# zkwebauthn/webauthn-halo2

Hardware: AMD Instinct MI355X
Metric: webauthn_es256_proofs_per_sec_k19 (higher is better)
Workload: dtype u256-montgomery (9x29-bit carry-free limbs in the hot kernels: bucket accumulation, NTT, reduction tails, quotient; 8x32-bit limbs elsewhere and in memory)

## Files before the change

include/zkmi355.h:

```cpp
#ifndef ZKMI355_H
#define ZKMI355_H

#include <stddef.h>
#include <stdint.h>

#ifdef __cplusplus
extern "C" {
#endif

#define ZK_OK 0
#define ZK_EINVAL (-1)
#define ZK_ENOMEM (-2)
#define ZK_EHIP (-3)
#define ZK_ENODEV (-4)
#define ZK_ESTATE (-5)
#define ZK_EWITNESS (-6)
#define ZK_EINTERNAL (-7)
#define ZK_ELAYOUT (-8)

typedef struct zk_ctx zk_ctx;
typedef uint64_t zk_poly;

#define ZK_BASIS_MONOMIAL 0
#define ZK_BASIS_LAGRANGE 1
// ... 4 lines not shown
void* zk_host_alloc(size_t bytes);
void zk_host_free(void* p);
int zk_ctx_create(int device_id, zk_ctx** out);
int zk_ctx_create_shared(zk_ctx* parent, zk_ctx** out);
void zk_ctx_destroy(zk_ctx* ctx);
const char* zk_strerror(int code);
int zk_last_hip_error(const zk_ctx* ctx);
int zk_sync(zk_ctx* ctx);
#define ZK_OPT_MSM_WINDOW 1
#define ZK_OPT_MSM_BATCH 2
#define ZK_OPT_NTT_MAX_RADIX_LOG2 3
#define ZK_OPT_GP_BATCH_INVERT 4
#define ZK_OPT_MSM_TAIL_STREAM 5
#define ZK_OPT_MSM_TAIL_MAIN_ABOVE 6
#define ZK_OPT_BATCH_PASS_COLUMNS 7
#define ZK_OPT_XFORM_STREAM 8
#define ZK_OPT_MSM_STREAM 9
#define ZK_OPT_MSM_T1 10
#define ZK_OPT_STREAM_AUDIT 11
#define ZK_OPT_STREAM_PRIORITY 12
#define ZK_OPT_QUOTIENT_DOMAIN 13
#define ZK_OPT_ACTIVITY_HOLD 14
int zk_ctx_set_option(zk_ctx* ctx, int option, int64_t value);

int zk_msm_bn254(zk_ctx* ctx, const uint64_t* scalars_mont ,
                 const uint64_t* bases_affine_mont , size_t n,
                 uint64_t out_jacobian_mont[12]);
int zk_msm_srs(zk_ctx* ctx, int basis , const uint64_t* scalars_mont , size_t n,
               uint64_t out_jacobian_mont[12]);
int zk_ntt_bn254_fr(zk_ctx* ctx, uint64_t* a_mont , const uint64_t omega_mont[4],
                    uint32_t log_n);

int zk_srs_setup(zk_ctx* ctx, uint32_t k, const uint8_t seed[32]);
int zk_srs_load(zk_ctx* ctx, uint32_t k, const uint64_t* g, const uint64_t* g_lagrange);
int zk_srs_export(zk_ctx* ctx, int basis, uint64_t* out_affine_mont , size_t first, size_t count);
int zk_srs_k(const zk_ctx* ctx);
int zk_srs_msm_plan(const zk_ctx* ctx, uint32_t* window_bits, uint32_t* windows);

#define ZK_SERDE_PROCESSED 0
#define ZK_SERDE_RAW_BYTES 1
#define ZK_SERDE_RAW_BYTES_UNCHECKED 2
int zk_srs_write(zk_ctx* ctx, int format, uint8_t* out, size_t cap, size_t* len);
int zk_srs_read(zk_ctx* ctx, const uint8_t* bytes, size_t len, int format);
int zk_srs_set_g2(zk_ctx* ctx, const uint64_t g2[16], const uint64_t s_g2[16]);

int zk_g_to_lagrange(zk_ctx* ctx, const uint64_t* g , uint32_t k, uint64_t* out );
// ... 225 lines not shown
```

webauthn-halo2_amd/csrc/ctx.h:

```cpp
#pragma once
#include <map>
#include <memory>
#include <new>
#include <mutex>
#include <unordered_map>
#include <vector>

#include "../../include/zkmi355.h"
#include "engine.h"
#include "activity.h"
#include "audit.h"
#include "hostutil.h"

using namespace zk;

struct zk_pk_rec;

struct PolyRec {
    Fr* ptr;
    size_t n;
};

struct SrsBlock {
    int device = -1;
// ... 30 lines not shown
    bool audit_fault = false;
    std::mutex mu;
    std::map<uint32_t, Fr*> twiddles;
    std::map<uint32_t, Fr*> coset_points;
    std::map<uint32_t, Fr*> twiddles_ntt;
    std::map<uint32_t, Fr> ninv;
    std::map<uint32_t, Fr*> twiddles_ninv;
    std::map<uint32_t, Fr*> coset3_pre;
    std::map<uint32_t, Coset3Consts> coset3_consts;
    uint32_t opt_verify_inst_eval = 0;
    uint32_t opt_quotient_domain = 0;
    uint64_t srs_gen = 0;
    uint32_t opt_msm_window = 0, opt_msm_batch = 0, opt_ntt_max_r = 0, opt_gp_batch_invert = 0;
    uint32_t opt_tail_stream = 0;
    uint32_t opt_tail_main_above = 0;
    uint32_t opt_batch_pass_cols = 0;
    uint32_t msm_min_cols = 0;
    activity::State act;
    hipStream_t tail_stream = nullptr;
    hipStream_t msm_stream = nullptr;
    hipEvent_t ev_msm_in = nullptr;
    bool msm_side = false;
    uint32_t opt_msm_stream = 0;
    uint32_t opt_msm_t1 = 0;
    hipStream_t xform_stream = nullptr;
    hipEvent_t ev_rows = nullptr, ev_xform = nullptr;
    bool xform_pending = false;
    uint32_t opt_xform_stream = 0;
    uint64_t stream_counts[4] = {0, 0, 0, 0};
    static constexpr int MSM_LANES = 3;
    struct MsmLane {
        MsmWorkspace* ws = nullptr;
        MsmWorkspace* ws_gen = nullptr;
        MsmWorkspace* ws_run = nullptr;
        hipStream_t tail = nullptr;
        hipEvent_t head_done = nullptr, tail_done = nullptr;
        hipEvent_t t_head[2] = {nullptr, nullptr};
        hipEvent_t t_acc[4] = {nullptr, nullptr, nullptr, nullptr};
        size_t n = 0;
        const G1Affine* table = nullptr;
        G1X* host_buf = nullptr;
        bool busy = false;
        uint32_t nwin = 0, cw = 0;
        uint32_t batch = 1;
        bool fixed = false;
    } lanes[MSM_LANES];
// ... 132 lines not shown
```

webauthn-halo2_amd/csrc/ctx.hip:

```cpp
#include <stdlib.h>

#include <algorithm>
#include <new>

#include "ctx.h"
#include "prover.h"

namespace zk {
G1Affine g1_jac_to_affine_host(const G1Jac& p) {
    G1Affine r;
    if (p.z.is_zero()) {
        r.x = Fq::zero();
        r.y = Fq::zero();
        return r;
    }
    const Fq zi = fe_inv_fast(p.z);
    const Fq zi2 = fe_sqr(zi);
    r.x = fe_mul(p.x, zi2);
    r.y = fe_mul(p.y, fe_mul(zi2, zi));
    return r;
}
}

int ctx_bind(zk_ctx* c) {
    hipError_t e = hipSetDevice(c->device);
    if (e != hipSuccess) {
        c->last_hip = (int)e;
        return ZK_EHIP;
    }
// ... 129 lines not shown
}

const char* zk_strerror(int code) {
    switch (code) {
        case ZK_OK: return "ok";
        case ZK_EINVAL: return "invalid argument";
        case ZK_ENOMEM: return "out of memory";
        case ZK_EHIP: return "HIP runtime error";
        case ZK_ENODEV: return "no usable gfx950 device";
        case ZK_ESTATE: return "missing prerequisite (SRS / key not loaded)";
        case ZK_EWITNESS: return "witness does not satisfy the circuit (lookup input outside the table)";
        case ZK_EINTERNAL: return "internal error (C++ exception stopped at the ABI boundary)";
        case ZK_ELAYOUT: return "selector columns outside the layout of compress_selectors the key is built for";
        default: return "unknown error";
    }
}

ZK_API(zk_ctx_create, (int device_id, zk_ctx** out), (device_id, out)) {
    if (!out) return ZK_EINVAL;
    if (int rc = device_id_ok(device_id)) return rc;
    zk_ctx* c = new (std::nothrow) zk_ctx();
    if (!c) return ZK_ENOMEM;
    c->device = device_id;
    if (hipSetDevice(device_id) != hipSuccess ||
        ((c->stream_slot = pool_take_slot(device_id, &c->stream)) < 0 && hipStreamCreate(&c->stream) != hipSuccess) ||
        hipHostMalloc(&c->host_small, 8 * sizeof(Fr)) != hipSuccess ||
        hipMalloc(&c->small, (2048 + 8) * sizeof(Fr)) != hipSuccess) {
        zk_ctx_destroy(c);
        return ZK_EHIP;
    }
    for (int i = 0; i < ZK_T_COUNT; i++)
        if (hipEventCreate(&c->ev[i][0]) != hipSuccess || hipEventCreate(&c->ev[i][1]) != hipSuccess) {
            zk_ctx_destroy(c);
            return ZK_EHIP;
        }
    bool ok = true;
    for (hipEvent_t* e : {&c->ev_msm_in, &c->ev_rows, &c->ev_xform}) ok = ok && hipEventCreateWithFlags(e, hipEventDisableTiming) == hipSuccess;
    for (int i = 0; i < zk_ctx::MSM_LANES && ok; i++) {
        zk_ctx::MsmLane& L = c->lanes[i];
        L.tail = c->stream;
        for (hipEvent_t& e : L.t_head) ok = ok && hipEventCreate(&e) == hipSuccess;
        for (hipEvent_t& e : L.t_acc) ok = ok && hipEventCreate(&e) == hipSuccess;
        for (hipEvent_t* e : {&L.head_done, &L.tail_done}) ok = ok && hipEventCreateWithFlags(e, hipEventDisableTiming) == hipSuccess;
        ok = ok && hipHostMalloc(&L.host_buf, (size_t)MSM_MAX_BATCH * 15 * 4 * sizeof(G1X)) == hipSuccess;
    }
    if (!ok) {
// ... 5 lines not shown
    ctx_activity_register(c);
    *out = c;
    return ZK_OK;
}

ZK_API(zk_ctx_create_shared, (zk_ctx* parent, zk_ctx** out), (parent, out)) {
    if (!parent || !out) return ZK_EINVAL;
    zk_ctx* c = nullptr;
    int rc = zk_ctx_create(parent->device, &c);
    if (rc) return rc;
    std::lock_guard<std::mutex> lk(parent->mu);
    if (parent->srs_k >= 0) {
        static_cast<SrsView&>(*c) = *parent;
        c->opt_msm_window = parent->opt_msm_window;
        c->opt_msm_batch = parent->opt_msm_batch;
        c->opt_ntt_max_r = parent->opt_ntt_max_r;
        c->opt_gp_batch_invert = parent->opt_gp_batch_invert;
        c->opt_tail_stream = parent->opt_tail_stream;
        c->opt_tail_main_above = parent->opt_tail_main_above;
        c->opt_batch_pass_cols = parent->opt_batch_pass_cols;
        c->opt_xform_stream = parent->opt_xform_stream;
        c->opt_msm_stream = parent->opt_msm_stream;
        c->opt_msm_t1 = parent->opt_msm_t1;
        c->srs_gen++;
    }
    *out = c;
    return ZK_OK;
}

void zk_ctx_destroy(zk_ctx* c) {
    if (!c) return;
    ctx_activity_unregister(c);
    hipSetDevice(c->device);
    if (c->stream) aud_sync(c, c->stream);
    if (c->tail_stream) aud_sync(c, c->tail_stream);
    if (c->xform_stream) aud_sync(c, c->xform_stream);
    if (c->msm_stream) aud_sync(c, c->msm_stream);
    for (auto& kv : c->twiddles) hipFree(kv.second);
    for (auto& kv : c->twiddles_ntt) hipFree(kv.second);
    for (auto& kv : c->twiddles_ninv) hipFree(kv.second);
    for (auto& kv : c->coset_points) hipFree(kv.second);
    for (auto& kv : c->coset3_pre) hipFree(kv.second);
    pk_destroy_all(c);
    for (auto& kv : c->polys) hipFree(kv.second.ptr);
    for (auto& r : c->poly_spare) hipFree(r.ptr);
    c->srs.reset();
// ... 128 lines not shown
    *total_ms = c->acc_ms[which];
    *count = c->acc_n[which];
    return ZK_OK;
}

namespace {
struct PlainOption {
    int option;
    int64_t min, max;
    uint32_t zk_ctx::*member;
};
const PlainOption PLAIN_OPTIONS[] = {
    {ZK_OPT_MSM_WINDOW, 9, 17, &zk_ctx::opt_msm_window},
    {ZK_OPT_MSM_TAIL_STREAM, 0, 2, &zk_ctx::opt_tail_stream},
    {ZK_OPT_MSM_TAIL_MAIN_ABOVE, 0, 64, &zk_ctx::opt_tail_main_above},
    {ZK_OPT_MSM_STREAM, 0, 2, &zk_ctx::opt_msm_stream},
    {ZK_OPT_MSM_T1, 0, 2, &zk_ctx::opt_msm_t1},
    {ZK_OPT_XFORM_STREAM, 0, 2, &zk_ctx::opt_xform_stream},
    {ZK_OPT_BATCH_PASS_COLUMNS, 0, MSM_MAX_BATCH, &zk_ctx::opt_batch_pass_cols},
    {ZK_OPT_MSM_BATCH, 0, MSM_MAX_BATCH, &zk_ctx::opt_msm_batch},
    {ZK_OPT_NTT_MAX_RADIX_LOG2, 1, 11, &zk_ctx::opt_ntt_max_r},
    {ZK_OPT_QUOTIENT_DOMAIN, 0, 2, &zk_ctx::opt_quotient_domain},
};
}

ZK_API(zk_ctx_set_option, (zk_ctx* c, int option, int64_t value), (c, option, value)) {
    if (!c || value < 0) return ZK_EINVAL;
    std::lock_guard<std::mutex> lk(c->mu);
    for (const PlainOption& o : PLAIN_OPTIONS)
        if (o.option == option) {
            if (value && (value < o.min || value > o.max)) return ZK_EINVAL;
            c->*o.member = (uint32_t)value;
            return ZK_OK;
        }
    switch (option) {
        case ZK_OPT_STREAM_AUDIT:
            if (value > 2) return ZK_EINVAL;
            c->audit.reset();
            c->audit.streams[0] = c->stream;
            c->audit.on = value != 0;
            c->audit_fault = value == 2;
            return ZK_OK;
        case ZK_OPT_GP_BATCH_INVERT:
            c->opt_gp_batch_invert = value ? 1 : 0;
            return ZK_OK;
        case ZK_OPT_ACTIVITY_HOLD:
// ... 27 lines not shown
```

webauthn-halo2_amd/csrc/pk.h:

```cpp
#pragma once
#include <utility>
#include <vector>

#include "ctx.h"
#include "prover.h"

inline int resolve_scheme(int transcript, int* scheme) {
    if (transcript != ZK_TRANSCRIPT_BLAKE2B && transcript != ZK_TRANSCRIPT_EVM) return ZK_EINVAL;
    if (*scheme == ZK_SCHEME_DEFAULT) *scheme = transcript == ZK_TRANSCRIPT_EVM ? ZK_SCHEME_GWC : ZK_SCHEME_SHPLONK;
    return *scheme == ZK_SCHEME_GWC || *scheme == ZK_SCHEME_SHPLONK ? ZK_OK : ZK_EINVAL;
}

enum ColType { COL_ADVICE = 0, COL_FIXED = 1, COL_INSTANCE = 2 };
struct Col {
    int type;
    uint32_t idx;
};

struct Layout {
    uint32_t k, n, A, L, F, lookup_bits, idle;
    uint32_t n_inst;
    bool single;
    uint32_t n_gate, n_lookup_cols, n_adv, fx_table, fx_qlookup, n_fix;
    std::vector<uint32_t> fx_sel;
// ... 73 lines not shown
static constexpr uint32_t BATCH_ARGS_MIN = 8;
static constexpr uint32_t ROWS_CAP = 512, ROWS_BLOCKS = 16;

struct zk_pk_rec {
    Layout lay;
    uint64_t srs_gen = 0;
    std::vector<Fr*> dev;
    std::vector<Fr*> fixed_val, fixed_poly, fixed_coset, sigma_val, sigma_poly, sigma_coset;
    Fr *l0_coset = nullptr, *l_last_coset = nullptr, *l_active_coset = nullptr;
    std::vector<Fr*> fixed_c3, sigma_c3;
    Fr *l0_c3 = nullptr, *l_last_c3 = nullptr, *l_active_c3 = nullptr;
    std::vector<G1Affine> fixed_commit, perm_commit;
    Fr transcript_repr;
    bool verify_only = false;
    G1Affine* d_vk_bases = nullptr;
    std::vector<Fr*> adv_val, adv_poly, adv_coset;
    Fr *inst_val = nullptr, *inst_poly = nullptr, *inst_coset = nullptr;
    std::vector<Fr*> z_val, z_poly, z_coset;
    std::vector<Fr*> lk_in, lk_ap, lk_ap_poly, lk_ap_coset, lk_sp, lk_sp_poly, lk_sp_coset, lk_z, lk_z_poly, lk_z_coset,
        lk_in_coset;
    Fr *random_poly = nullptr, *h_ext = nullptr, *h_comb = nullptr;
    Fr *t_num = nullptr, *t_den = nullptr, *t_frac = nullptr, *t_a = nullptr, *t_b = nullptr, *t_small = nullptr;
    Fr* kd_scratch = nullptr;
    Fr* tail_host = nullptr;
    RowEntry* rows_host = nullptr;
    RowEntry* rows_dev = nullptr;
    LookupScratch lks{};
    uint32_t* lk_u32 = nullptr;
    std::vector<Fr*> gp_num, gp_den, gp_loc_p, gp_loc_r;
    Fr* gp_tot = nullptr;
    Fr* gp_scal = nullptr;
    Fr* gp_host = nullptr;
    GpItem* d_gp_items = nullptr;
    void *h_batch_args = nullptr, *d_batch_args = nullptr;
    size_t batch_args_bytes = 0;
    QuotientArgs* d_qargs = nullptr;
    QuotientArgs* h_qargs = nullptr;
    EvalItem *d_evargs = nullptr, *h_evargs = nullptr;
    Fr t_inv[4];
    bool t_inv_ready = false;
    uint32_t max_evals = 0;
    LcTerm *d_lc_terms = nullptr, *h_lc_terms = nullptr;
    uint32_t lc_cap = 0, lc_used = 0;
    Fr *ev_scratch = nullptr, *ev_out = nullptr;
    bool is_member = false;
    std::vector<zk_pk_rec*> members;
// ... 61 lines not shown
```

webauthn-halo2_amd/csrc/prover.hip:

```cpp
#include <stdlib.h>

#include <algorithm>
#include <deque>
#include <functional>
#include <memory>
#include <unordered_map>
#include <vector>

#include "prover_steps.h"

using namespace zk;

#ifdef ZK_HOST_TRACE
#include <chrono>
#include <cstdio>
static std::chrono::steady_clock::time_point& ht_last() {
    static thread_local std::chrono::steady_clock::time_point t = std::chrono::steady_clock::now();
    return t;
}
#define HT(name)                                                                                                  \
    do {                                                                                                          \
        const auto ht_now = std::chrono::steady_clock::now();                                                     \
        fprintf(stderr, "HT %-24s +%7.1f us\n", name, std::chrono::duration<double, std::micro>(ht_now - ht_last()).count()); \
        ht_last() = ht_now;                                                                                       \
    } while (0)
#else
#define HT(name) do { } while (0)
#endif


namespace {
// ... 580 lines not shown
    }

    struct CR {
        const Fr* poly;
        std::vector<int> rots;
        std::vector<Fr> evals;
    };
    struct RotPt {
        int rot;
        Fr pt, canon;
    };
    struct RS {
        std::vector<int> rots;
        std::vector<size_t> coms;
    };
    struct Shplonk {
        std::vector<CR> com;
        std::vector<RotPt> rot_pts;
        std::vector<RS> rsets;
        std::vector<int> all_rots;
        std::vector<std::vector<Fr>> low;
        Fr yc, v;
        Fr* hx = nullptr;
    };
    static const RotPt& sh_rot_pt(const Shplonk& S, int r) {
        for (auto& e : S.rot_pts)
            if (e.rot == r) return e;
        return S.rot_pts[0];
    }
    int shplonk_stage1(const std::vector<Q>& queries, const Fr& x, Shplonk& S) {
        std::vector<CR>& com = S.com;
        {
            std::unordered_map<const Fr*, size_t> seen;
            seen.reserve(queries.size());
            for (auto& qq : queries) {
                auto it = seen.find(qq.poly);
                if (it == seen.end()) {
                    it = seen.emplace(qq.poly, com.size()).first;
                    com.push_back(CR{qq.poly, {}, {}});
                }
                com[it->second].rots.push_back(qq.rot);
                com[it->second].evals.push_back(qq.eval);
            }
        }
        for (auto& qq : queries) {
            bool have = false;
// ... 22 lines not shown
                r2.push_back(cr.rots[i]);
                e2.push_back(cr.evals[i]);
            }
            cr.rots = r2;
            cr.evals = e2;
            for (int r : cr.rots)
                if (std::find(all_rots.begin(), all_rots.end(), r) == all_rots.end()) all_rots.push_back(r);
            size_t hit = rsets.size();
            for (size_t si = 0; si < rsets.size(); si++)
                if (rsets[si].rots == cr.rots) hit = si;
            if (hit == rsets.size()) rsets.push_back(RS{cr.rots, {}});
            rsets[hit].coms.push_back(ci);
        }
        std::sort(all_rots.begin(), all_rots.end(), pt_less);
        HT("grouped");
        S.yc = tr->squeeze();
        S.v = tr->squeeze();
        const Fr yc = S.yc, v = S.v;
        S.low.assign(com.size(), {});
        Fr* hx = pk->t_frac;
        S.hx = hx;
        Fr* sbuf[6] = {pk->h_ext, pk->h_ext + n, pk->h_ext + 2 * (size_t)n, pk->h_ext + 3 * (size_t)n, pk->t_num, pk->t_den};
        if (rsets.size() > 6) return ZK_ESTATE;
        std::vector<std::vector<Fr>> set_pts;
        size_t max_pts = 0;
        for (size_t si = 0; si < rsets.size(); si++) {
            auto& rs = rsets[si];
            std::vector<Fr> pts;
            for (int r : rs.rots) pts.push_back(sh_rot_pt(S, r).pt);
            const std::vector<std::vector<Fr>> basis = lagrange_basis(pts);
            std::vector<Term> terms;
            std::vector<Fr> rsum(pts.size(), Fr::zero());
            Fr py = Fr::one();
            for (size_t ci : rs.coms) {
                const CR& cr = com[ci];
                std::vector<Fr>& lo = S.low[ci];
                lo.assign(pts.size(), Fr::zero());
                for (size_t j = 0; j < pts.size(); j++)
                    for (size_t t = 0; t < pts.size(); t++) lo[t] = fe_add(lo[t], fe_mul(basis[j][t], cr.evals[j]));
                terms.push_back(Term{cr.poly, py});
                for (size_t t = 0; t < pts.size(); t++) rsum[t] = fe_add(rsum[t], fe_mul(py, lo[t]));
                py = fe_mul(py, yc);
            }
            if (pts.size() > 8) return ZK_ESTATE;
            lincomb_many(sbuf[si], terms, false, Fr::zero(), false, &rsum);
        HT("set lincomb launched");
            max_pts = std::max(max_pts, pts.size());
            set_pts.push_back(pts);
        }
        for (size_t step = 0; step < max_pts; step++) {
            Fr* bufs[6];
            Fr zs[6];
            uint32_t cnt = 0;
            for (size_t si = 0; si < rsets.size(); si++)
                if (step < set_pts[si].size()) {
                    bufs[cnt] = sbuf[si];
                    zs[cnt] = set_pts[si][step];
                    cnt++;
                }
            if (c->audit.on) {
                std::vector<const void*> b(bufs, bufs + cnt);
                AV(b, b, "SHPLONK: division step");
            }
            launch_kate_division_batch(bufs, bufs, zs, cnt, n, pk->kd_scratch, st);
        }
        {
            std::vector<Term> terms;
            Fr pv = Fr::one();
            for (size_t si = 0; si < rsets.size(); si++) {
                terms.push_back(Term{sbuf[si], pv});
                pv = fe_mul(pv, v);
            }
            lincomb_many(hx, terms, false, Fr::zero());
        HT("hx launched");
        }
        return rc;
    }
    int shplonk_stage2(Shplonk& S, const Fr** out) {
        const Fr u = tr->squeeze();
        HT("u squeezed");
        std::vector<Term> terms;
        Fr sub = Fr::zero();
        Fr pv = Fr::one();
        std::vector<Fr> z_diffs;
        for (auto& rs : S.rsets) {
            std::vector<Fr> diffs;
            for (int r : S.all_rots)
                if (std::find(rs.rots.begin(), rs.rots.end(), r) == rs.rots.end()) diffs.push_back(sh_rot_pt(S, r).pt);
            const Fr zi = vanishing_eval(diffs, u);
            z_diffs.push_back(zi);
            Fr py = Fr::one();
            for (size_t ci : rs.coms) {
                const Fr coef = fe_mul(fe_mul(pv, zi), py);
                terms.push_back(Term{S.com[ci].poly, coef});
                sub = fe_add(sub, fe_mul(coef, eval_small(S.low[ci], u)));
                py = fe_mul(py, S.yc);
            }
            pv = fe_mul(pv, S.v);
        }
        std::vector<Fr> all_pts;
        for (int r : S.all_rots) all_pts.push_back(sh_rot_pt(S, r).pt);
        const Fr zt = vanishing_eval(all_pts, u);
        terms.push_back(Term{S.hx, fe_neg(zt)});
        lincomb_many(pk->t_a, terms, true, sub);
        HT("L launched");
        A({pk->t_a}, {pk->t_b}, "SHPLONK: final division");
        launch_kate_division(pk->t_a, pk->t_b, n, u, pk->kd_scratch, st);
        A({pk->t_b}, {pk->t_b}, "SHPLONK: scale");
        launch_scale(pk->t_b, fe_inv_fast(z_diffs[0]), n, st);
        *out = pk->t_b;
        return rc;
    }
    int open_shplonk(const std::vector<Q>& queries, const Fr& x) {
        Shplonk S;
        if (int r = shplonk_stage1(queries, x, S)) return r;
        commit_write(S.hx, ZK_BASIS_MONOMIAL);
        if (!ok()) return rc;
        const Fr* last = nullptr;
        if (int r = shplonk_stage2(S, &last)) return r;
        commit_write(last, ZK_BASIS_MONOMIAL);
        return rc;
    }
};

#include "prover_lockstep.h"

}

namespace {
struct ProveQuiesce {
    zk_ctx* c;
    explicit ProveQuiesce(zk_ctx* ctx) : c(ctx) { ctx_activity_hold(c, true); }
// ... 234 lines not shown
```

webauthn-halo2_amd/csrc/prover_key.hip:

```cpp
#include <stdlib.h>

#include <algorithm>
#include <unordered_map>
#include <vector>

#include "pk.h"
#include "vkrepr.h"

using namespace zk;

namespace {

__global__ void sigma_kernel(const uint2* __restrict__ map, const Fr* __restrict__ tw, const Fr* __restrict__ dpow,
                             Fr* __restrict__ out, uint32_t n) {
    const uint32_t i = blockIdx.x * blockDim.x + threadIdx.x;
    if (i >= n) return;
    const uint2 m = map[i];
    fe_store(out + i, fe_mul(fe_load(dpow + m.x), fe_load(tw + m.y)));
}

bool commit(zk_ctx* c, const Fr* poly, size_t len, int basis, G1Affine* out) {
    G1Jac j;
    if (ctx_msm_device(c, poly, ctx_basis(c, basis), len, &j) != ZK_OK) return false;
    *out = g1_jac_to_affine_host(j);
// ... 84 lines not shown
    }
    for (uint32_t l = 0; l < lay.n_lookups; l++) {
        pk->lk_in.push_back(lay.single ? d.alloc(n) : nullptr);
        pk->lk_ap.push_back(d.alloc(n));
        pk->lk_ap_poly.push_back(d.alloc(n));
        pk->lk_ap_coset.push_back(d.alloc(N));
        pk->lk_sp.push_back(d.alloc(n));
        pk->lk_sp_poly.push_back(d.alloc(n));
        pk->lk_sp_coset.push_back(d.alloc(N));
        pk->lk_z.push_back(d.alloc(n));
        pk->lk_z_poly.push_back(d.alloc(n));
        pk->lk_z_coset.push_back(d.alloc(N));
    }
    pk->random_poly = d.alloc(n);
    pk->h_ext = d.alloc(N);
    pk->h_comb = d.alloc(n);
    pk->t_num = d.alloc(n);
    pk->t_den = d.alloc(n);
    pk->t_frac = d.alloc(n);
    pk->t_a = d.alloc(n);
    pk->t_b = d.alloc(n);
    pk->t_small = d.alloc(n / 16 + 8192);
    pk->kd_scratch = d.alloc((size_t)KD_MAX_BATCH * kate_division_scratch(n));
    {
        const uint32_t nprod = lay.n_chunks + lay.n_lookups;
        for (uint32_t p = 0; p < nprod; p++) {
            pk->gp_num.push_back(d.alloc(n));
            pk->gp_den.push_back(d.alloc(n));
            pk->gp_loc_p.push_back(d.alloc(n));
            pk->gp_loc_r.push_back(d.alloc(n));
        }
        pk->gp_tot = d.alloc((size_t)2 * gp_blocks(n) * nprod);
        pk->gp_scal = d.alloc((size_t)4 * nprod);
        if (hipHostMalloc(&pk->gp_host, (size_t)2 * nprod * sizeof(Fr)) != hipSuccess ||
            hipMalloc(&pk->d_gp_items, nprod * sizeof(GpItem)) != hipSuccess)
            return fail(ZK_ENOMEM);
    }
    if (d.rc) return fail(d.rc);
    if (hipHostMalloc(&pk->tail_host, (pk->max_evals + 16) * sizeof(Fr)) != hipSuccess) return fail(ZK_ENOMEM);
    if (hipHostMalloc(&pk->rows_host, (size_t)ROWS_BLOCKS * ROWS_CAP * sizeof(RowEntry)) != hipSuccess ||
        hipMalloc(&pk->rows_dev, (size_t)ROWS_BLOCKS * ROWS_CAP * sizeof(RowEntry)) != hipSuccess)
        return fail(ZK_ENOMEM);
    if (hipHostMalloc(&pk->h_evargs, pk->max_evals * sizeof(EvalItem)) != hipSuccess ||
        hipMalloc(&pk->d_evargs, pk->max_evals * sizeof(EvalItem)) != hipSuccess)
        return fail(ZK_ENOMEM);
    pk->lc_cap = 2 * (pk->max_evals + 8);
// ... 24 lines not shown
        bytes = std::max(bytes, (size_t)lay.n_lookups * sizeof(LkNumDenArgs));
        bytes = std::max(bytes, (size_t)lay.n_adv * sizeof(CopyPair));
        pk->batch_args_bytes = bytes;
        if (hipMalloc(&pk->d_batch_args, bytes) != hipSuccess || hipHostMalloc(&pk->h_batch_args, bytes) != hipSuccess) return fail(ZK_ENOMEM);
    }
    return ZK_OK;
}

static zk_pk_rec* pk_make_member(zk_ctx* c, const zk_pk_rec* pk) {
    zk_pk_rec* m = new (std::nothrow) zk_pk_rec(*pk);
    if (!m) return nullptr;
    m->is_member = true;
    m->dev.clear();
    m->members.clear();
    m->bb = nullptr;
    m->wc = nullptr;
    m->pc = nullptr;
    for (auto* v : {&m->adv_val, &m->adv_poly, &m->adv_coset, &m->z_val, &m->z_poly, &m->z_coset, &m->lk_in, &m->lk_ap, &m->lk_ap_poly,
                    &m->lk_ap_coset, &m->lk_sp, &m->lk_sp_poly, &m->lk_sp_coset, &m->lk_z, &m->lk_z_poly, &m->lk_z_coset, &m->lk_in_coset,
                    &m->gp_num, &m->gp_den, &m->gp_loc_p, &m->gp_loc_r})
        v->clear();
    m->inst_val = m->inst_poly = m->inst_coset = nullptr;
    m->random_poly = m->h_ext = m->h_comb = m->t_num = m->t_den = m->t_frac = m->t_a = m->t_b = m->t_small = m->kd_scratch = nullptr;
    m->tail_host = nullptr;
    m->rows_host = m->rows_dev = nullptr;
    m->lk_u32 = nullptr;
    m->gp_tot = m->gp_scal = m->gp_host = nullptr;
    m->d_gp_items = nullptr;
    m->h_batch_args = m->d_batch_args = nullptr;
    m->d_qargs = m->h_qargs = nullptr;
    m->d_evargs = m->h_evargs = nullptr;
    m->d_lc_terms = m->h_lc_terms = nullptr;
    m->ev_scratch = m->ev_out = nullptr;
    m->lc_used = 0;
    if (pk_alloc_workspace(c, m) != ZK_OK) {
        pk_destroy(m);
        return nullptr;
    }
    return m;
}

int pk_ensure_batch(zk_ctx* c, zk_pk_rec* pk, uint32_t batch) {
    if (batch <= 1) return ZK_OK;
    const Layout& lay = pk->lay;
    const uint32_t n = lay.n, T = 1u << lay.lookup_bits, nprod = lay.n_chunks + lay.n_lookups;
    if ((pk->members.size() + 1 < batch || !pk->bb || pk->bb->cap < batch) && !c->poly_spare.empty()) ctx_release_spares(c);
// ... 574 lines not shown
```

webauthn-halo2_amd/ecdsa_p256.py:

```python
import dataclasses
import hashlib
import os
import queue
import threading
import time

import numpy as np

from . import circuit
from .engine import (ZK_PK_CHECK_ALL, ZK_SCHEME_GWC, ZK_SCHEME_SHPLONK, ZK_SERDE_RAW_BYTES, ZK_SRS_CONTRIB_LINKS,
                     ZK_SRS_CONTRIB_NONTRIVIAL, ZK_SRS_CONTRIB_RESIDENT, ZK_SRS_CONTRIB_SAME_SECRET, ZK_TRANSCRIPT_BLAKE2B,
                     ZK_ES256_BATCH_MAX, ZK_TRANSCRIPT_EVM, Engine, ZkError, stream_placement)

_STATE = {}
_SLOTS_LOCK = threading.Lock()
_STATE_LOCK = threading.RLock()
PIPELINES_PER_DEVICE = 4
_MAX_SLOT_SETS = 4
_PIPELINE_BYTES = {17: 2.0 * 2**30, 18: 3.2 * 2**30, 19: 5.3 * 2**30, 20: 10.5 * 2**30, 21: 21.0 * 2**30}


def pipelines_for(degree: int, device: int = 0) -> int:
    from .engine import device_mem_info

    want = max(1, PIPELINES_PER_DEVICE)
    per = _PIPELINE_BYTES.get(degree, _PIPELINE_BYTES[21] * (1 << max(0, degree - 21)) if degree > 21 else _PIPELINE_BYTES[17])
    per += _MAX_SLOT_SETS * 32 * (1 << degree)
    try:
        free, _ = device_mem_info(device)
    except Exception:
        return want
    return max(1, min(want, int(0.75 * free // per)))


def _config_for(degree: int) -> circuit.CircuitParams:
    path = os.environ.get("ECDSA_CONFIG")
    if path and os.path.exists(path):
        p = circuit.CircuitParams.from_json(open(path).read().strip().splitlines()[0])
        if p.degree == degree:
            return p
    if degree == 19:
        return circuit.K19
# ... 638 lines not shown
```

webauthn-halo2_amd/engine.py:

```python
import ctypes
import os

import numpy as np

_HERE = os.path.dirname(os.path.abspath(__file__))
_LIB = None

ZK_BASIS_MONOMIAL = 0
ZK_BASIS_LAGRANGE = 1
ZK_T_MSM, ZK_T_NTT, ZK_T_QUOTIENT, ZK_T_EVAL, ZK_T_MSM_ACCUM, ZK_T_MSM_COLUMNS, ZK_T_MSM_TAIL_MAIN, ZK_T_MSM_TAIL = 0, 1, 2, 3, 4, 5, 6, 7


ZK_TRANSCRIPT_BLAKE2B, ZK_TRANSCRIPT_EVM = 0, 1
ZK_SERDE_PROCESSED, ZK_SERDE_RAW_BYTES, ZK_SERDE_RAW_BYTES_UNCHECKED = 0, 1, 2
ZK_OPT_MSM_WINDOW, ZK_OPT_MSM_BATCH, ZK_OPT_NTT_MAX_RADIX_LOG2, ZK_OPT_GP_BATCH_INVERT, ZK_OPT_MSM_TAIL_STREAM = 1, 2, 3, 4, 5
ZK_OPT_MSM_TAIL_MAIN_ABOVE, ZK_OPT_BATCH_PASS_COLUMNS, ZK_OPT_XFORM_STREAM, ZK_OPT_MSM_STREAM, ZK_OPT_MSM_T1, ZK_OPT_STREAM_AUDIT = 6, 7, 8, 9, 10, 11
ZK_OPT_STREAM_PRIORITY, ZK_OPT_QUOTIENT_DOMAIN, ZK_OPT_ACTIVITY_HOLD = 12, 13, 14
ZK_VERIFY_INSTANCE_EVAL_AUTO, ZK_VERIFY_INSTANCE_EVAL_HOST, ZK_VERIFY_INSTANCE_EVAL_DEVICE = 0, 1, 2
ZK_SCHEME_DEFAULT, ZK_SCHEME_GWC, ZK_SCHEME_SHPLONK = 0, 1, 2
ZK_VERIFY_BATCH_MAX = 1024
ZK_PROVE_MULTI_MAX = 16
ZK_ES256_VALID, ZK_ES256_RANGE, ZK_ES256_OFF_CURVE, ZK_ES256_MISMATCH = 0, 1, 2, 3
ZK_ES256_BATCH_MAX = 16384
ZK_SRS_CHECK_POWERS, ZK_SRS_CHECK_LAGRANGE, ZK_SRS_CHECK_GENERATORS = 1, 2, 4
# ... 107 lines not shown
    if _LIB is not None:
        return _LIB
    p = lib_path()
    if not os.path.exists(p):
        raise ZkError(-4, f"{p} is missing — run ./build.sh (no CPU fallback exists)")
    L = ctypes.CDLL(p)
    u64p = ctypes.POINTER(ctypes.c_uint64)
    vp = ctypes.c_void_p
    sz = ctypes.c_size_t
    u32 = ctypes.c_uint32
    sig = {
        "zk_device_count": ([], ctypes.c_int),
        "zk_device_pci_bus_id": ([ctypes.c_int, ctypes.c_char_p, sz], ctypes.c_int),
        "zk_device_mem_info": ([ctypes.c_int, ctypes.POINTER(ctypes.c_size_t), ctypes.POINTER(ctypes.c_size_t)], ctypes.c_int),
        "zk_host_alloc": ([sz], vp),
        "zk_host_free": ([vp], None),
        "zk_ctx_create": ([ctypes.c_int, ctypes.POINTER(vp)], ctypes.c_int),
        "zk_ctx_create_shared": ([vp, ctypes.POINTER(vp)], ctypes.c_int),
        "zk_ctx_destroy": ([vp], None),
        "zk_strerror": ([ctypes.c_int], ctypes.c_char_p),
        "zk_last_hip_error": ([vp], ctypes.c_int),
        "zk_sync": ([vp], ctypes.c_int),
        "zk_ctx_set_option": ([vp, ctypes.c_int, ctypes.c_int64], ctypes.c_int),
        "zk_msm_bn254": ([vp, u64p, u64p, sz, u64p], ctypes.c_int),
        "zk_msm_srs": ([vp, ctypes.c_int, u64p, sz, u64p], ctypes.c_int),
        "zk_ntt_bn254_fr": ([vp, u64p, u64p, u32], ctypes.c_int),
        "zk_srs_setup": ([vp, u32, ctypes.c_char_p], ctypes.c_int),
        "zk_srs_load": ([vp, u32, u64p, u64p], ctypes.c_int),
        "zk_srs_export": ([vp, ctypes.c_int, u64p, sz, sz], ctypes.c_int),
        "zk_srs_k": ([vp], ctypes.c_int),
        "zk_srs_msm_plan": ([vp, ctypes.POINTER(u32), ctypes.POINTER(u32)], ctypes.c_int),
        "zk_poly_alloc": ([vp, sz, ctypes.POINTER(ctypes.c_uint64)], ctypes.c_int),
        "zk_poly_free": ([vp, ctypes.c_uint64], ctypes.c_int),
        "zk_poly_detach": ([vp, ctypes.c_uint64, ctypes.POINTER(ctypes.c_uint64)], ctypes.c_int),
        "zk_poly_attach": ([vp, ctypes.c_uint64, ctypes.POINTER(ctypes.c_uint64)], ctypes.c_int),
        "zk_poly_discard": ([ctypes.c_uint64], ctypes.c_int),
        "zk_poly_len": ([vp, ctypes.c_uint64, ctypes.POINTER(sz)], ctypes.c_int),
        "zk_poly_upload": ([vp, ctypes.c_uint64, u64p, sz], ctypes.c_int),
        "zk_poly_download": ([vp, ctypes.c_uint64, u64p, sz], ctypes.c_int),
        "zk_poly_copy": ([vp, ctypes.c_uint64, ctypes.c_uint64], ctypes.c_int),
        "zk_commit": ([vp, ctypes.c_uint64, ctypes.c_int, u64p], ctypes.c_int),
        "zk_commit_batch": ([vp, ctypes.POINTER(ctypes.c_uint64), sz, ctypes.c_int, u64p], ctypes.c_int),
        "zk_lagrange_to_coeff": ([vp, ctypes.c_uint64], ctypes.c_int),
        "zk_coeff_to_lagrange": ([vp, ctypes.c_uint64], ctypes.c_int),
        "zk_coeff_to_extended": ([vp, ctypes.c_uint64, ctypes.c_uint64], ctypes.c_int),
        "zk_extended_to_coeff": ([vp, ctypes.c_uint64, sz], ctypes.c_int),
# ... 68 lines not shown
        "zk_quotient_multi": ([vp, ctypes.c_uint64, sz, ctypes.POINTER(ctypes.c_uint64), sz, ctypes.POINTER(ctypes.c_uint64),
                               ctypes.POINTER(ctypes.c_uint64), sz, ctypes.POINTER(ctypes.c_uint64), sz, u64p, u64p, u64p, ctypes.c_int,
                               ctypes.c_uint64], ctypes.c_int),
        "zk_eval_batch": ([vp, ctypes.POINTER(ctypes.c_uint64), u64p, sz, u64p], ctypes.c_int),
        "zk_pk_export_poly": ([vp, ctypes.c_uint64, ctypes.c_int, sz, ctypes.c_uint64], ctypes.c_int),
        "zk_random_poly": ([vp, ctypes.c_char_p, ctypes.c_uint64, ctypes.c_uint64], ctypes.c_int),
        "zk_vk_read": ([vp, ctypes.POINTER(CircuitParamsC), vp, sz, ctypes.c_int, u64p, ctypes.POINTER(ctypes.c_uint64)], ctypes.c_int),
        "zk_vk_from_parts": ([vp, ctypes.POINTER(CircuitParamsC), u64p, u64p, u64p, ctypes.POINTER(ctypes.c_uint64)], ctypes.c_int),
        "zk_verify": ([vp, ctypes.c_uint64, ctypes.c_int, ctypes.c_int, ctypes.c_char_p, sz, ctypes.POINTER(ctypes.c_int)], ctypes.c_int),
        "zk_verify_batch": ([vp, ctypes.c_uint64, sz, ctypes.c_int, ctypes.c_int, ctypes.POINTER(ctypes.c_char_p), ctypes.POINTER(sz),
                             ctypes.POINTER(ctypes.c_uint8)], ctypes.c_int),
        "zk_witness_check": ([vp, ctypes.c_uint64, ctypes.POINTER(ctypes.c_uint64), sz, ctypes.POINTER(WitnessFailureC), sz,
                              ctypes.POINTER(ctypes.c_uint64)], ctypes.c_int),
        "zk_pk_check": ([vp, ctypes.c_uint64, ctypes.POINTER(u32), ctypes.POINTER(PkFindingC), sz, ctypes.POINTER(sz)], ctypes.c_int),
        "zk_stream_placement": ([ctypes.c_int, ctypes.c_int, ctypes.POINTER(PlacementC)], ctypes.c_int),
        "zk_ctx_stream_info": ([vp, ctypes.POINTER(CtxStreamsC)], ctypes.c_int),
    }
    for name, (args, res) in sig.items():
        fn = getattr(L, name, None)
        if fn is None:
            if name in ("zk_witness_check", "zk_pk_check", "zk_stream_placement", "zk_ctx_stream_info", "zk_proof_size_multi",
                        "zk_prove_multi", "zk_verify_multi", "zk_prove_public", "zk_verify_public", "zk_witness_check_public",
                        "zk_pk_num_instance_columns", "zk_prove_batch_public", "zk_prove_multi_public", "zk_verify_batch_public",
                        "zk_verify_multi_public", "zk_instance_eval", "zk_verify_instance_eval_mode", "zk_es256_verify") and os.environ.get("ZKMI355_LIB"):
                continue
            raise ZkError(-4, f"{p} does not export {name} — rebuild it (./build.sh)")
        fn.argtypes = args
        fn.restype = res
    _LIB = L
    return L


def _p(a):
    return a.ctypes.data_as(ctypes.POINTER(ctypes.c_uint64))


def _arr(a, cols):
    a = np.ascontiguousarray(a, dtype=np.uint64)
    if a.size % cols:
        raise ValueError("bad array shape")
    return a.reshape(-1, cols)


class Poly:

    def __init__(self, eng, handle, n):
        self.eng, self.h, self.n = eng, handle, n
# ... 14 lines not shown
        else:
            rc = self.L.zk_ctx_create(device, ctypes.byref(ctx))
        if rc != 0:
            raise ZkError(rc, "zk_ctx_create: " + self.L.zk_strerror(rc).decode())
        self.ctx = ctx

    def close(self):
        if getattr(self, "ctx", None):
            self.L.zk_ctx_destroy(self.ctx)
            self.ctx = None

    def __del__(self):
        try:
            self.close()
        except Exception:
            pass

    def _chk(self, rc, what):
        if rc != 0:
            raise ZkError(rc, what + ": " + self.L.zk_strerror(rc).decode(), self.L.zk_last_hip_error(self.ctx))

    def set_option(self, option, value):
        self._chk(self.L.zk_ctx_set_option(self.ctx, option, value), "zk_ctx_set_option")

    def msm_srs(self, scalars_mont, basis):
        s = _arr(scalars_mont, 4)
        out = np.zeros(12, dtype=np.uint64)
        self._chk(self.L.zk_msm_srs(self.ctx, basis, _p(s), s.shape[0], _p(out)), "zk_msm_srs")
        return out

    def msm(self, scalars_mont, bases_mont):
        s = _arr(scalars_mont, 4)
        b = _arr(bases_mont, 8)
        if s.shape[0] != b.shape[0]:
            raise ValueError("scalars / bases length mismatch")
        out = np.zeros(12, dtype=np.uint64)
        self._chk(self.L.zk_msm_bn254(self.ctx, _p(s), _p(b), s.shape[0], _p(out)), "zk_msm_bn254")
        return out

    def ntt(self, a_mont, omega_mont, log_n):
        a = _arr(a_mont, 4).copy()
        if a.shape[0] != (1 << log_n):
            raise ValueError("length != 2^log_n")
        w = np.ascontiguousarray(omega_mont, dtype=np.uint64).reshape(4)
        self._chk(self.L.zk_ntt_bn254_fr(self.ctx, _p(a), _p(w), log_n), "zk_ntt_bn254_fr")
        return a
# ... 616 lines not shown
```

Before: 105.6.

## Restructure SHPLONK opening to divide once per evaluation point via partial fractions

Adds a per-point SHPLONK route, on by default, used when there are at most six rotation points. Each rotation set's combined polynomial is split across its evaluation points with partial-fraction coefficients, so one batched Kate division runs per distinct point. This replaces the per-set, per-step division loop. The final scale by the inverse of the first vanishing factor is folded into the lincomb coefficients, which drops one launch. The cost is six extra n-sized device buffers per proving key and raised pipeline memory estimates.

```diff
diff --git a/include/zkmi355.h b/include/zkmi355.h
--- a/include/zkmi355.h
+++ b/include/zkmi355.h
@@ -50,6 +50,7 @@
 #define ZK_OPT_QUOTIENT_DOMAIN 13
 #define ZK_OPT_ACTIVITY_HOLD 14
 int zk_ctx_set_option(zk_ctx* ctx, int option, int64_t value);
+int zk_ctx_set_open_route(zk_ctx* ctx, int route);
 
 int zk_msm_bn254(zk_ctx* ctx, const uint64_t* scalars_mont ,
                  const uint64_t* bases_affine_mont , size_t n,
diff --git a/webauthn-halo2_amd/csrc/ctx.h b/webauthn-halo2_amd/csrc/ctx.h
--- a/webauthn-halo2_amd/csrc/ctx.h
+++ b/webauthn-halo2_amd/csrc/ctx.h
@@ -76,6 +76,7 @@
     hipEvent_t ev_msm_in = nullptr;
     bool msm_side = false;
     uint32_t opt_msm_stream = 0;
+    uint32_t opt_open_route = 0;
     uint32_t opt_msm_t1 = 0;
     hipStream_t xform_stream = nullptr;
     hipEvent_t ev_rows = nullptr, ev_xform = nullptr;
diff --git a/webauthn-halo2_amd/csrc/ctx.hip b/webauthn-halo2_amd/csrc/ctx.hip
--- a/webauthn-halo2_amd/csrc/ctx.hip
+++ b/webauthn-halo2_amd/csrc/ctx.hip
@@ -5,6 +5,10 @@
 
 #include "ctx.h"
 #include "prover.h"
+
+#ifndef ZK_OPEN_ROUTE_DEFAULT
+#define ZK_OPEN_ROUTE_DEFAULT 0
+#endif
 
 namespace zk {
 G1Affine g1_jac_to_affine_host(const G1Jac& p) {
@@ -180,6 +184,7 @@
     zk_ctx* c = new (std::nothrow) zk_ctx();
     if (!c) return ZK_ENOMEM;
     c->device = device_id;
+    c->opt_open_route = ZK_OPEN_ROUTE_DEFAULT;
     if (hipSetDevice(device_id) != hipSuccess ||
         ((c->stream_slot = pool_take_slot(device_id, &c->stream)) < 0 && hipStreamCreate(&c->stream) != hipSuccess) ||
         hipHostMalloc(&c->host_small, 8 * sizeof(Fr)) != hipSuccess ||
@@ -231,6 +236,7 @@
         c->opt_xform_stream = parent->opt_xform_stream;
         c->opt_msm_stream = parent->opt_msm_stream;
         c->opt_msm_t1 = parent->opt_msm_t1;
+        c->opt_open_route = parent->opt_open_route;
         c->srs_gen++;
     }
     *out = c;
@@ -405,6 +411,13 @@
     {ZK_OPT_NTT_MAX_RADIX_LOG2, 1, 11, &zk_ctx::opt_ntt_max_r},
     {ZK_OPT_QUOTIENT_DOMAIN, 0, 2, &zk_ctx::opt_quotient_domain},
 };
+}
+
+ZK_API(zk_ctx_set_open_route, (zk_ctx* c, int route), (c, route)) {
+    if (!c || route < 0 || route > 1) return ZK_EINVAL;
+    std::lock_guard<std::mutex> lk(c->mu);
+    c->opt_open_route = (uint32_t)route;
+    return ZK_OK;
 }
 
 ZK_API(zk_ctx_set_option, (zk_ctx* c, int option, int64_t value), (c, option, value)) {
diff --git a/webauthn-halo2_amd/csrc/open_route.h b/webauthn-halo2_amd/csrc/open_route.h
--- /dev/null
+++ b/webauthn-halo2_amd/csrc/open_route.h
@@ -0,0 +1,18 @@
+#pragma once
+#include <vector>
+
+#include "hostutil.h"
+
+namespace zk {
+
+inline std::vector<Fr> partial_fraction_coeffs(const std::vector<Fr>& pts) {
+    const size_t m = pts.size();
+    std::vector<Fr> den(m, Fr::one()), inv(m);
+    for (size_t j = 0; j < m; j++)
+        for (size_t i = 0; i < m; i++)
+            if (i != j) den[j] = fe_mul(den[j], fe_sub(pts[j], pts[i]));
+    fr_batch_invert(den.data(), inv.data(), (uint32_t)m);
+    return inv;
+}
+
+}
diff --git a/webauthn-halo2_amd/csrc/pk.h b/webauthn-halo2_amd/csrc/pk.h
--- a/webauthn-halo2_amd/csrc/pk.h
+++ b/webauthn-halo2_amd/csrc/pk.h
@@ -119,6 +119,7 @@
     Fr *random_poly = nullptr, *h_ext = nullptr, *h_comb = nullptr;
     Fr *t_num = nullptr, *t_den = nullptr, *t_frac = nullptr, *t_a = nullptr, *t_b = nullptr, *t_small = nullptr;
     Fr* kd_scratch = nullptr;
+    Fr* open_f[6] = {nullptr, nullptr, nullptr, nullptr, nullptr, nullptr};
     Fr* tail_host = nullptr;
     RowEntry* rows_host = nullptr;
     RowEntry* rows_dev = nullptr;
diff --git a/webauthn-halo2_amd/csrc/prover.hip b/webauthn-halo2_amd/csrc/prover.hip
--- a/webauthn-halo2_amd/csrc/prover.hip
+++ b/webauthn-halo2_amd/csrc/prover.hip
@@ -7,6 +7,7 @@
 #include <unordered_map>
 #include <vector>
 
+#include "open_route.h"
 #include "prover_steps.h"
 
 using namespace zk;
@@ -633,6 +634,9 @@
         std::vector<std::vector<Fr>> low;
         Fr yc, v;
         Fr* hx = nullptr;
+        bool per_point = false;
+        std::vector<const Fr*> F;
+        std::vector<std::vector<Fr>> rem;
     };
     static const RotPt& sh_rot_pt(const Shplonk& S, int r) {
         for (auto& e : S.rot_pts)
@@ -701,6 +705,7 @@
         S.hx = hx;
         Fr* sbuf[6] = {pk->h_ext, pk->h_ext + n, pk->h_ext + 2 * (size_t)n, pk->h_ext + 3 * (size_t)n, pk->t_num, pk->t_den};
         if (rsets.size() > 6) return ZK_ESTATE;
+        S.per_point = c->opt_open_route == 0 && all_rots.size() <= 6;
         std::vector<std::vector<Fr>> set_pts;
         size_t max_pts = 0;
         for (size_t si = 0; si < rsets.size(); si++) {
@@ -722,11 +727,22 @@
                 py = fe_mul(py, yc);
             }
             if (pts.size() > 8) return ZK_ESTATE;
-            lincomb_many(sbuf[si], terms, false, Fr::zero(), false, &rsum);
+            if (S.per_point) {
+                if (terms.size() == 1) {
+                    S.F.push_back(terms[0].poly);
+                } else {
+                    lincomb_many(pk->open_f[si], terms, false, Fr::zero());
+                    S.F.push_back(pk->open_f[si]);
+                }
+                S.rem.push_back(rsum);
+            } else {
+                lincomb_many(sbuf[si], terms, false, Fr::zero(), false, &rsum);
+            }
         HT("set lincomb launched");
             max_pts = std::max(max_pts, pts.size());
             set_pts.push_back(pts);
         }
+        if (S.per_point) return shplonk_per_point(S, set_pts, sbuf);
         for (size_t step = 0; step < max_pts; step++) {
             Fr* bufs[6];
             Fr zs[6];
@@ -755,6 +771,41 @@
         }
         return rc;
     }
+    int shplonk_per_point(Shplonk& S, const std::vector<std::vector<Fr>>& set_pts, Fr* const qbuf[6]) {
+        const size_t np = S.all_rots.size();
+        std::vector<std::vector<Term>> g(np);
+        Fr pv = Fr::one();
+        for (size_t si = 0; si < S.rsets.size(); si++) {
+            const std::vector<Fr> cz = partial_fraction_coeffs(set_pts[si]);
+            for (size_t j = 0; j < cz.size(); j++) {
+                const size_t pi = std::find(S.all_rots.begin(), S.all_rots.end(), S.rsets[si].rots[j]) - S.all_rots.begin();
+                g[pi].push_back(Term{S.F[si], fe_mul(pv, cz[j])});
+            }
+            pv = fe_mul(pv, S.v);
+        }
+        const Fr* src[6];
+        Fr* dst[6];
+        Fr zs[6];
+        std::vector<Term> sum;
+        for (size_t pi = 0; pi < np; pi++) {
+            zs[pi] = sh_rot_pt(S, S.all_rots[pi]).pt;
+            dst[pi] = qbuf[pi];
+            if (g[pi].size() == 1) {
+                src[pi] = g[pi][0].poly;
+                sum.push_back(Term{qbuf[pi], g[pi][0].c});
+            } else {
+                lincomb_many(qbuf[pi], g[pi], false, Fr::zero());
+                src[pi] = qbuf[pi];
+                sum.push_back(Term{qbuf[pi], Fr::one()});
+            }
+        }
+        HT("point lincombs launched");
+        if (c->audit.on) AV(std::vector<const void*>(src, src + np), std::vector<const void*>(dst, dst + np), "SHPLONK: division by (X - point)");
+        launch_kate_division_batch(src, dst, zs, (uint32_t)np, n, pk->kd_scratch, st);
+        lincomb_many(S.hx, sum, false, Fr::zero());
+        HT("hx launched");
+        return rc;
+    }
     int shplonk_stage2(Shplonk& S, const Fr** out) {
         const Fr u = tr->squeeze();
         HT("u squeezed");
@@ -762,12 +813,20 @@
         Fr sub = Fr::zero();
         Fr pv = Fr::one();
         std::vector<Fr> z_diffs;
-        for (auto& rs : S.rsets) {
+        for (size_t si = 0; si < S.rsets.size(); si++) {
+            const RS& rs = S.rsets[si];
             std::vector<Fr> diffs;
             for (int r : S.all_rots)
                 if (std::find(rs.rots.begin(), rs.rots.end(), r) == rs.rots.end()) diffs.push_back(sh_rot_pt(S, r).pt);
             const Fr zi = vanishing_eval(diffs, u);
             z_diffs.push_back(zi);
+            if (S.per_point) {
+                const Fr coef = fe_mul(pv, zi);
+                terms.push_back(Term{S.F[si], coef});
+                sub = fe_add(sub, fe_mul(coef, eval_small(S.rem[si], u)));
+                pv = fe_mul(pv, S.v);
+                continue;
+            }
             Fr py = Fr::one();
             for (size_t ci : rs.coms) {
                 const Fr coef = fe_mul(fe_mul(pv, zi), py);
@@ -781,12 +840,19 @@
         for (int r : S.all_rots) all_pts.push_back(sh_rot_pt(S, r).pt);
         const Fr zt = vanishing_eval(all_pts, u);
         terms.push_back(Term{S.hx, fe_neg(zt)});
+        const Fr z0_inv = fe_inv_fast(z_diffs[0]);
+        if (S.per_point) {
+            for (Term& t : terms) t.c = fe_mul(t.c, z0_inv);
+            sub = fe_mul(sub, z0_inv);
+        }
         lincomb_many(pk->t_a, terms, true, sub);
         HT("L launched");
         A({pk->t_a}, {pk->t_b}, "SHPLONK: final division");
         launch_kate_division(pk->t_a, pk->t_b, n, u, pk->kd_scratch, st);
-        A({pk->t_b}, {pk->t_b}, "SHPLONK: scale");
-        launch_scale(pk->t_b, fe_inv_fast(z_diffs[0]), n, st);
+        if (!S.per_point) {
+            A({pk->t_b}, {pk->t_b}, "SHPLONK: scale");
+            launch_scale(pk->t_b, z0_inv, n, st);
+        }
         *out = pk->t_b;
         return rc;
     }
diff --git a/webauthn-halo2_amd/csrc/prover_key.hip b/webauthn-halo2_amd/csrc/prover_key.hip
--- a/webauthn-halo2_amd/csrc/prover_key.hip
+++ b/webauthn-halo2_amd/csrc/prover_key.hip
@@ -130,6 +130,7 @@
     pk->t_b = d.alloc(n);
     pk->t_small = d.alloc(n / 16 + 8192);
     pk->kd_scratch = d.alloc((size_t)KD_MAX_BATCH * kate_division_scratch(n));
+    for (Fr*& f : pk->open_f) f = d.alloc(n);
     {
         const uint32_t nprod = lay.n_chunks + lay.n_lookups;
         for (uint32_t p = 0; p < nprod; p++) {
@@ -200,6 +201,7 @@
         v->clear();
     m->inst_val = m->inst_poly = m->inst_coset = nullptr;
     m->random_poly = m->h_ext = m->h_comb = m->t_num = m->t_den = m->t_frac = m->t_a = m->t_b = m->t_small = m->kd_scratch = nullptr;
+    for (Fr*& f : m->open_f) f = nullptr;
     m->tail_host = nullptr;
     m->rows_host = m->rows_dev = nullptr;
     m->lk_u32 = nullptr;
diff --git a/webauthn-halo2_amd/ecdsa_p256.py b/webauthn-halo2_amd/ecdsa_p256.py
--- a/webauthn-halo2_amd/ecdsa_p256.py
+++ b/webauthn-halo2_amd/ecdsa_p256.py
@@ -17,7 +17,7 @@
 _STATE_LOCK = threading.RLock()
 PIPELINES_PER_DEVICE = 4
 _MAX_SLOT_SETS = 4
-_PIPELINE_BYTES = {17: 2.0 * 2**30, 18: 3.2 * 2**30, 19: 5.3 * 2**30, 20: 10.5 * 2**30, 21: 21.0 * 2**30}
+_PIPELINE_BYTES = {17: 2.1 * 2**30, 18: 3.3 * 2**30, 19: 5.4 * 2**30, 20: 10.7 * 2**30, 21: 21.4 * 2**30}
 
 
 def pipelines_for(degree: int, device: int = 0) -> int:
diff --git a/webauthn-halo2_amd/engine.py b/webauthn-halo2_amd/engine.py
--- a/webauthn-halo2_amd/engine.py
+++ b/webauthn-halo2_amd/engine.py
@@ -153,6 +153,7 @@
         "zk_last_hip_error": ([vp], ctypes.c_int),
         "zk_sync": ([vp], ctypes.c_int),
         "zk_ctx_set_option": ([vp, ctypes.c_int, ctypes.c_int64], ctypes.c_int),
+        "zk_ctx_set_open_route": ([vp, ctypes.c_int], ctypes.c_int),
         "zk_msm_bn254": ([vp, u64p, u64p, sz, u64p], ctypes.c_int),
         "zk_msm_srs": ([vp, ctypes.c_int, u64p, sz, u64p], ctypes.c_int),
         "zk_ntt_bn254_fr": ([vp, u64p, u64p, u32], ctypes.c_int),
@@ -267,7 +268,8 @@
             if name in ("zk_witness_check", "zk_pk_check", "zk_stream_placement", "zk_ctx_stream_info", "zk_proof_size_multi",
                         "zk_prove_multi", "zk_verify_multi", "zk_prove_public", "zk_verify_public", "zk_witness_check_public",
                         "zk_pk_num_instance_columns", "zk_prove_batch_public", "zk_prove_multi_public", "zk_verify_batch_public",
-                        "zk_verify_multi_public", "zk_instance_eval", "zk_verify_instance_eval_mode", "zk_es256_verify") and os.environ.get("ZKMI355_LIB"):
+                        "zk_verify_multi_public", "zk_instance_eval", "zk_verify_instance_eval_mode", "zk_es256_verify",
+                        "zk_ctx_set_open_route") and os.environ.get("ZKMI355_LIB"):
                 continue
             raise ZkError(-4, f"{p} does not export {name} — rebuild it (./build.sh)")
         fn.argtypes = args
@@ -328,6 +330,9 @@
 
     def set_option(self, option, value):
         self._chk(self.L.zk_ctx_set_option(self.ctx, option, value), "zk_ctx_set_option")
+
+    def set_open_route(self, route):
+        self._chk(self.L.zk_ctx_set_open_route(self.ctx, route), "zk_ctx_set_open_route")
 
     def msm_srs(self, scalars_mont, basis):
         s = _arr(scalars_mont, 4)
```

After: 106.4 (median of 5 runs). About the same (+0.8%).
